# tensorboy/pytorch_Realtime_Multi-Person_Pose_Estimation

Hardware: AMD Instinct MI355X
Metric: end-to-end persons-posed FPS at 368x368 (net+pafprocess) (higher is better)
Workload: dtype fp32; 1 GPU; rtpose VGG19 368x368 batch=32 synthetic images, single MI355X, fp32 (BASELINE.json configs[1]); per-GPU batch 32, one process per GPU; global_batch=32, weights=seeded He init (no checkpoint offline), decoder_input=synthetic scene + 1e-3 * net output (blend kernel timed), humans_per_batch=163, parallelism=single GPU

## Files before the change

### pytorch_realtime_multi-person_pose_estimation_amd/csrc/conv_wino4.hip

```cpp
#include <hip/hip_runtime.h>

#include <cmath>
#include <cstdio>
#include <cstdlib>
#include <type_traits>

#include "conv_desc.h"
#include "launchers.h"
#include "wino_common.h"

namespace rtpose {

namespace wino4 {

using namespace winoc;

constexpr int W4_L0 = 6;

typedef float floatx4 __attribute__((ext_vector_type(4)));

struct Group {
  const float* in;
  const float* w;
  const float* bias;
  float* out;
  int in_cstride, in_choff, in_ws, in_hs, in_lead;
  int out_cstride, out_choff, out_ws, out_hs, out_lead;
  int cout, cout_pad;
  int in_pq, out_pq;
  size_t in_bytes, w_bytes, out_bytes;
};

__device__ __forceinline__ int px_floats(int cstride, int pq) { return pq ? 8 : cstride; }
__device__ __forceinline__ size_t ch0_floats(int choff, int pq) { return pq ? (size_t)(choff >> 3) * pq * 8 + (choff & 7) : choff; }
__device__ __forceinline__ unsigned col_floats(int col, int pq) { return pq ? (unsigned)(col >> 3) * pq * 8 + (col & 7) : col; }

struct Args {
  Group g[2];
  int N, H, W;
  int TY, TX, T;
  int cin;
  int relu, pool;
  int mtiles, ntiles, ncombo, xcd_remap;
  int persist;
  int mt0;
};

struct ArgsP : Args {
  const float* prelu[2];
};
template <bool PR>
using ArgsT = typename std::conditional<PR, ArgsP, Args>::type;
template <bool PR>
__device__ __forceinline__ float slope_of(const ArgsT<PR>& A, int grp, int ncol, int cout) {
  if constexpr (PR) return ncol < cout ? (grp ? A.prelu[1] : A.prelu[0])[ncol] : 0.f;
  return 0.f;
}

constexpr int NT = 32;
constexpr int NC = 64;
constexpr int CK = 8;
constexpr int NFP = 18;
constexpr int NPW = 9;
constexpr int NFW = 18;
constexpr int NB = 6;
constexpr int PF = 5;
constexpr int VBUF = NFP * 4 * NT;
constexpr int UBUF = 36 * 2 * NT;
static_assert((2 * NPW) % NB == 0, "the B ring rotates in step with two chunks");

template <class Out>
__device__ __forceinline__ void bt6(const F4 (&d)[6], Out out) {
  out(0, fma4(1.265625f, d[0], fma4(-2.8125f, d[2], d[4])));
  __builtin_amdgcn_sched_barrier(0);
  {
    const F4 e1 = fma4(-2.25f, d[2], d[4]), o1 = fma4(-2.25f, d[1], d[3]);
    out(1, fma4(0.75f, o1, e1));
    out(2, fma4(-0.75f, o1, e1));
  }
  __builtin_amdgcn_sched_barrier(0);
  {
    const F4 e2 = fma4(-0.5625f, d[2], d[4]), o2 = fma4(-0.5625f, d[1], d[3]);
    out(3, fma4(1.5f, o2, e2));
    out(4, fma4(-1.5f, o2, e2));
  }
  __builtin_amdgcn_sched_barrier(0);
  out(5, fma4(1.265625f, d[1], fma4(-2.8125f, d[3], d[5])));
}

__device__ __forceinline__ f2 splat(float s) { return f2{s, s}; }
__device__ __forceinline__ void at4_lo(const f2 (&m)[6], f2& y0, f2& y1) {
  const f2 s12 = m[1] + m[2], d12 = m[1] - m[2], s34 = m[3] + m[4], d34 = m[3] - m[4];
  y0 = (m[0] + s12) + s34;
  y1 = __builtin_elementwise_fma(splat(1.5f), d34, splat(0.75f) * d12);
}
__device__ __forceinline__ void at4_hi(const f2 (&m)[6], f2& y2, f2& y3) {
  const f2 s12 = m[1] + m[2], d12 = m[1] - m[2], s34 = m[3] + m[4], d34 = m[3] - m[4];
  y2 = __builtin_elementwise_fma(splat(2.25f), s34, splat(0.5625f) * s12);
  y3 = __builtin_elementwise_fma(splat(3.375f), d34, splat(0.421875f) * d12) + m[5];
}

template <int RT, bool PR = false>
__global__ __launch_bounds__(512, 1) void wino4_f32(const ArgsT<PR> A) {
  constexpr int NT = 16 * RT;
  constexpr int VBUF = NFP * 4 * NT;
  constexpr int UBUF = 36 * 2 * NT;
  extern __shared__ __attribute__((aligned(16))) float4 L4[];
  auto Vb = [&](int i) -> float4* { return L4 + i * (VBUF + UBUF); };
  auto Ub = [&](int i) -> float4* { return L4 + (1 - i) * (VBUF + UBUF) + VBUF; };
  const int tid = threadIdx.x;
  const int lane = tid & 63;
  const int wv = __builtin_amdgcn_readfirstlane(tid >> 6);
  const int wn = wv & 3, fh = wv >> 2;
  const int r16 = lane & 15, kq = lane >> 4;

  const int bi = blockIdx.x;
  int j0, jstep, c;
  if (A.persist) {
    const int xcd = bi & 7, idx = bi >> 3;
    c = idx % A.ncombo;
    j0 = (idx / A.ncombo) * 8 + xcd;
    jstep = gridDim.x / A.ncombo;
  } else {
    if (A.xcd_remap) {
      const int xcd = bi & 7, j = bi >> 3;
      c = j % A.ncombo;
      j0 = (j / A.ncombo) * 8 + xcd;
    } else {
      j0 = bi % A.mtiles;
      c = bi / A.mtiles;
    }
    jstep = A.mtiles;
  }
  if (j0 >= A.mtiles) return;
  const int nt = c % A.ntiles, grp = c / A.ntiles;
  const Group g = grp ? A.g[1] : A.g[0];
  const int TT = A.TY * A.TX;

  const bool s1 = RT == 2 ? wv < 6 : wv < 3, s2 = RT == 2 ? wv >= 2 : (wv >= 3 && wv < 6);
  const int turn = wv >> 2;
  const int wl1 = RT == 2 ? lane >> 1 : (lane >> 1) & 15, cg1 = lane & 1;
  const int wl = RT == 2 ? lane & 31 : lane & 15, cg = RT == 2 ? lane >> 5 : (lane >> 4) & 1;
  const int py = RT == 2 ? wv : 2 * (s1 ? wv : 0) + (lane >> 5);
  const int fx = RT == 2 ? max(wv - 2, 0) : 2 * (s2 ? wv - 3 : 0) + (lane >> 5);
  const i32x4 rw = make_rsrc(g.w, g.w_bytes);
  const i32x4 rnull = make_rsrc(g.in, 0);
  i32x4 rin;
  unsigned pv[4];
  int lt = j0, lc = 3;
  const int cs_ld = px_floats(g.in_cstride, g.in_pq);
  const unsigned pxb = (unsigned)cs_ld * 4;
  const unsigned ckb = g.in_pq ? (unsigned)g.in_pq * (CK * 4) : CK * 4;
  const size_t in_ch0 = ch0_floats(g.in_choff, g.in_pq);
  auto set_loader = [&](int mt, i32x4& r_, unsigned (&v_)[4]) {
    size_t q0;
    {
      const int t = min((A.mt0 + mt) * NT, A.T - 1);
      const int n = t / TT, r = t - n * TT;
      const int ty = r / A.TX, tx = r - ty * A.TX;
      q0 = (size_t)g.in_lead + (size_t)(n * g.in_hs + 4 * ty - 1) * g.in_ws + (4 * tx - 1);
    }
    const int t = min((A.mt0 + mt) * NT + wl1, A.T - 1);
    const int n = t / TT, r = t - n * TT;
    const int ty = r / A.TX, tx = r - ty * A.TX;
    const int yy = min(4 * ty - 1 + py, A.H);
    const size_t qq = (size_t)g.in_lead + (size_t)(n * g.in_hs + yy) * g.in_ws + (4 * tx - 1);
    const size_t o0 = q0 * cs_ld + in_ch0;
    r_ = make_rsrc(g.in + o0, g.in_bytes - o0 * 4);
    v_[0] = (unsigned)(((qq - q0) * cs_ld + cg1 * 4) * 4);
#pragma unroll
    for (int n5 = 3; n5 < 6; ++n5) v_[n5 - 2] = v_[0] + (unsigned)min(n5, A.W + 1 - 4 * tx) * pxb;
  };
  F4 p[6];
  auto load_piece = [&](const i32x4& r_, const unsigned (&v_)[4], int chunk, int n5) {
    const unsigned cb = (unsigned)chunk * ckb;
    p[n5] = n5 < 3 ? bload(r_, v_[0], cb + n5 * pxb) : bload(r_, v_[n5 - 2], cb);
  };
  const int ust = (py * 2 + cg1) * NT + (wl1 ^ (4 * cg1));
  const int uld = ((fx * 6) * 2 + cg) * NT + (wl ^ (4 * cg));
  const int vst = ((fx * 3) * 4 + 2 * cg) * NT + wl;
  auto stage1 = [&](int ubuf) {
    float4* dst = Ub(ubuf) + ust;
    bt6(p, [&](int f, F4 u) { dst[f * 6 * 2 * NT] = to_float4(u); });
  };
  F4 q[6];
  auto stage2_read = [&](int ubuf) {
    const float4* src = Ub(ubuf) + uld;
#pragma unroll
    for (int y = 0; y < 6; ++y) {
      const float4 t = src[y * 2 * NT];
      q[y] = F4{f2{t.x, t.y}, f2{t.z, t.w}};
    }
  };
  auto stage2 = [&](int vbuf) {
    float4* dst = Vb(vbuf) + vst;
    F4 ev;
    bt6(q, [&](int f, F4 v) {
      if (f & 1) {
        dst[(f >> 1) * 4 * NT] = make_float4(ev.lo.x, ev.lo.y, v.lo.x, v.lo.y);
        dst[(f >> 1) * 4 * NT + NT] = make_float4(ev.hi.x, ev.hi.y, v.hi.x, v.hi.y);
      } else {
        ev = v;
      }
    });
  };

  const int ncol = nt * NC + wn * 16 + r16;
  floatx4 acc[NFW][RT];
  const float bias0 = g.bias[ncol];
  const float slope0 = slope_of<PR>(A, grp, ncol, g.cout);
  const unsigned boff = (unsigned)((kq * g.cout_pad + ncol) * 16);
  const unsigned fstep = (unsigned)(4 * g.cout_pad * 16);
  const unsigned wbase = (unsigned)fh * (NPW * fstep);
  unsigned wso = wbase;
  float4 bs[NB];
  const int nchunks = A.cin / CK;
  const int aoff = fh * NPW * 4 * NT + kq * NT + r16;

  set_loader(j0, rin, pv);
#pragma unroll
  for (int i = 0; i < 6; ++i) load_piece(rin, pv, 0, i);
  if (s1) stage1(0);
#pragma unroll
  for (int i = 0; i < 6; ++i) load_piece(rin, pv, 1, i);
#pragma unroll
  for (int f = 0; f < PF; ++f) {
    bs[f] = bload_f4(rw, boff, wso);
    wso += fstep;
  }
  __syncthreads();
  stage2_read(0);
  if (s2) stage2(0);
  if (s1) stage1(1);
#pragma unroll
  for (int i = 0; i < 6; ++i) load_piece(rin, pv, 2, i);
  __syncthreads();

#define RTPOSE_PIN()             \
  asm volatile("" ::: "memory"); \
  __builtin_amdgcn_sched_barrier(0)
  for (int mt = j0; mt < A.mtiles; mt += jstep) {
#pragma unroll
    for (int f = 0; f < NFW; ++f)
#pragma unroll
      for (int rt = 0; rt < RT; ++rt)
#pragma unroll
        for (int v = 0; v < 4; ++v) acc[f][rt][v] = 0.f;

    float4 a0, a1;
#pragma unroll 1
    for (int c2 = 0; c2 < nchunks; c2 += 2) {
#pragma unroll
      for (int h = 0; h < 2; ++h) {
        const float4* va = Vb(h) + aoff;
        if (lc == nchunks) {
          lc = 0;
          lt += jstep;
          if (lt < A.mtiles) set_loader(lt, rin, pv);
        }
        const int c3 = lc++;
        const i32x4 rl = s1 ? rin : rnull;
        a0 = va[RT == 2 ? fh * 16 : 0];
        if (RT == 2) a1 = va[(fh ^ 1) * 16];
#pragma unroll
        for (int i = 0; i < NPW; ++i) {
          const float4 bv = bs[(h * NPW + i) % NB];
          acc[2 * i][0] = __builtin_amdgcn_mfma_f32_16x16x4f32(a0.x, bv.x, acc[2 * i][0], 0, 0, 0);
          acc[2 * i + 1][0] = __builtin_amdgcn_mfma_f32_16x16x4f32(a0.z, bv.z, acc[2 * i + 1][0], 0, 0, 0);
          acc[2 * i][0] = __builtin_amdgcn_mfma_f32_16x16x4f32(a0.y, bv.y, acc[2 * i][0], 0, 0, 0);
          acc[2 * i + 1][0] = __builtin_amdgcn_mfma_f32_16x16x4f32(a0.w, bv.w, acc[2 * i + 1][0], 0, 0, 0);
          RTPOSE_PIN();
          if (i < NPW - 1) a0 = va[(i + 1) * 4 * NT + (RT == 2 ? fh * 16 : 0)];
          {
            const int L = h * NPW + i + PF;
            bs[L % NB] = bload_f4(rw, boff, wso);
            if (L % NPW == NPW - 1) wso = (c2 + L / NPW == nchunks - 1) ? wbase : wso + (NPW + 1) * fstep;
            else wso += fstep;
          }
          RTPOSE_PIN();
          if (RT == 2) {
            acc[2 * i][RT - 1] = __builtin_amdgcn_mfma_f32_16x16x4f32(a1.x, bv.x, acc[2 * i][RT - 1], 0, 0, 0);
            acc[2 * i + 1][RT - 1] = __builtin_amdgcn_mfma_f32_16x16x4f32(a1.z, bv.z, acc[2 * i + 1][RT - 1], 0, 0, 0);
            acc[2 * i][RT - 1] = __builtin_amdgcn_mfma_f32_16x16x4f32(a1.y, bv.y, acc[2 * i][RT - 1], 0, 0, 0);
            acc[2 * i + 1][RT - 1] = __builtin_amdgcn_mfma_f32_16x16x4f32(a1.w, bv.w, acc[2 * i + 1][RT - 1], 0, 0, 0);
          }
          RTPOSE_PIN();
          if (RT == 2 && i < NPW - 1) a1 = va[(i + 1) * 4 * NT + (fh ^ 1) * 16];
          if (i < 2) {
            if (s1 && i == turn) stage1(h);
          } else if (i < 4) {
            if (i == 2 + turn) stage2_read(h ^ 1);
          } else if (i < 6) {
            if (s2 && i == 4 + turn) stage2(h ^ 1);
          }
          if (i >= W4_L0 && i < W4_L0 + 3) {
            load_piece(rl, pv, c3, 2 * (i - W4_L0));
            load_piece(rl, pv, c3, 2 * (i - W4_L0) + 1);
          }
          RTPOSE_PIN();
        }
        __syncthreads();
      }
    }

    f2 sk[3][RT][4], sr[3][RT][4];
    if (RT == 2) {
      float4* const E = L4 + VBUF + UBUF;
#pragma unroll
      for (int vp = 0; vp < RT; ++vp) {
        f2 sg[3][4];
#pragma unroll
        for (int xl = 0; xl < 3; ++xl) {
          f2 m[6];
#pragma unroll
          for (int y = 0; y < 6; ++y) m[y] = f2{acc[xl * 6 + y][RT - 1][2 * vp], acc[xl * 6 + y][RT - 1][2 * vp + 1]};
          at4_lo(m, sg[xl][0], sg[xl][1]);
          at4_hi(m, sg[xl][2], sg[xl][3]);
        }
#pragma unroll
        for (int xl = 0; xl < 3; ++xl)
#pragma unroll
          for (int hh = 0; hh < 2; ++hh)
            E[(wv * 6 + xl * 2 + hh) * 64 + lane] =
                make_float4(sg[xl][2 * hh].x, sg[xl][2 * hh].y, sg[xl][2 * hh + 1].x, sg[xl][2 * hh + 1].y);
#pragma unroll
        for (int xl = 0; xl < 3; ++xl) {
          f2 m[6];
#pragma unroll
          for (int y = 0; y < 6; ++y) m[y] = f2{acc[xl * 6 + y][0][2 * vp], acc[xl * 6 + y][0][2 * vp + 1]};
          at4_lo(m, sk[xl][vp][0], sk[xl][vp][1]);
          at4_hi(m, sk[xl][vp][2], sk[xl][vp][3]);
        }
        __syncthreads();
#pragma unroll
        for (int xl = 0; xl < 3; ++xl)
#pragma unroll
          for (int hh = 0; hh < 2; ++hh) {
            const float4 t = E[((wv ^ 4) * 6 + xl * 2 + hh) * 64 + lane];
            sr[xl][vp][2 * hh] = f2{t.x, t.y};
            sr[xl][vp][2 * hh + 1] = f2{t.z, t.w};
          }
        __syncthreads();
      }
    } else {
      float4* const E = L4;
      auto rowsums = [&](int pair, f2 (&dst)[3][RT][4]) {
#pragma unroll
        for (int xl = 0; xl < 3; ++xl) {
          f2 m[6];
#pragma unroll
          for (int y = 0; y < 6; ++y)
            m[y] = pair ? f2{acc[xl * 6 + y][0][2], acc[xl * 6 + y][0][3]} : f2{acc[xl * 6 + y][0][0], acc[xl * 6 + y][0][1]};
          at4_lo(m, dst[xl][0][0], dst[xl][0][1]);
          at4_hi(m, dst[xl][0][2], dst[xl][0][3]);
        }
      };
      rowsums(fh ^ 1, sr);
#pragma unroll
      for (int xl = 0; xl < 3; ++xl)
#pragma unroll
        for (int hh = 0; hh < 2; ++hh)
          E[(wv * 6 + xl * 2 + hh) * 64 + lane] =
              make_float4(sr[xl][0][2 * hh].x, sr[xl][0][2 * hh].y, sr[xl][0][2 * hh + 1].x, sr[xl][0][2 * hh + 1].y);
      rowsums(fh, sk);
      __syncthreads();
#pragma unroll
      for (int xl = 0; xl < 3; ++xl)
#pragma unroll
        for (int hh = 0; hh < 2; ++hh) {
          const float4 t = E[((wv ^ 4) * 6 + xl * 2 + hh) * 64 + lane];
          sr[xl][0][2 * hh] = f2{t.x, t.y};
          sr[xl][0][2 * hh + 1] = f2{t.z, t.w};
        }
    }
    auto finish = [&](auto fhc) {
      constexpr int FH = decltype(fhc)::value;
      auto S = [&](int x, int vp, int i) -> f2 { return (x / 3 == FH) ? sk[x % 3][vp][i] : sr[x % 3][vp][i]; };
      const bool col_ok = ncol < g.cout;
      const int sc = A.pool ? 2 : 4;
      auto wt_q = [&](int n, int ty, int tx) -> int { return (n * g.out_hs + sc * ty) * g.out_ws + sc * tx; };
      int q0;
      {
        const int t = min((A.mt0 + mt) * NT, A.T - 1);
        const int n = t / TT, r = t - n * TT;
        const int ty = r / A.TX;
        q0 = wt_q(n, ty, r - ty * A.TX);
      }
      const int cs_st = px_floats(g.out_cstride, g.out_pq);
      const size_t oo0 = ((size_t)g.out_lead + (size_t)q0) * cs_st + ch0_floats(g.out_choff, g.out_pq);
      const i32x4 rout = make_rsrc(g.out + oo0, g.out_bytes - oo0 * 4);
      const unsigned cs4 = (unsigned)cs_st * 4, row4 = (unsigned)g.out_ws * cs4;
      const unsigned col4 = col_floats(ncol, g.out_pq) * 4;
      int tcur = (A.mt0 + mt) * NT + (RT == 2 ? FH * 16 + 4 * kq : 4 * kq + 2 * FH);
      int sn = tcur / TT, sy, sx;
      {
        const int r = tcur - sn * TT;
        sy = r / A.TX;
        sx = r - sy * A.TX;
      }
#pragma unroll
      for (int vp = 0; vp < RT; ++vp) {
        unsigned off[2];
        bool okv[2];
        int ylim[2], xlim[2];
#pragma unroll
        for (int e = 0; e < 2; ++e) {
          okv[e] = col_ok && tcur < A.T;
          off[e] = (unsigned)(wt_q(sn, sy, sx) - q0) * cs4 + col4;
          ylim[e] = A.H - 4 * sy;
          xlim[e] = A.W - 4 * sx;
          ++tcur;
          const bool wx = sx + 1 >= A.TX, wy = wx && sy + 1 >= A.TY;
          sx = wx ? 0 : sx + 1;
          sy = wy ? 0 : (wx ? sy + 1 : sy);
          sn += wy ? 1 : 0;
        }
#pragma unroll
        for (int ih = 0; ih < 2; ++ih) {
          f2 yy[2][4];
#pragma unroll
          for (int il = 0; il < 2; ++il) {
            f2 m[6];
#pragma unroll
            for (int x = 0; x < 6; ++x) m[x] = S(x, vp, 2 * ih + il);
            at4_lo(m, yy[il][0], yy[il][1]);
            at4_hi(m, yy[il][2], yy[il][3]);
          }
          if (A.pool) {
#pragma unroll
            for (int jh = 0; jh < 2; ++jh) {
              f2 mx = __builtin_elementwise_max(__builtin_elementwise_max(yy[0][2 * jh], yy[0][2 * jh + 1]),
                                                __builtin_elementwise_max(yy[1][2 * jh], yy[1][2 * jh + 1]));
              mx = mx + splat(bias0);
              if (A.relu) mx = __builtin_elementwise_max(mx, splat(0.f));
#pragma unroll
              for (int e = 0; e < 2; ++e) {
                const bool ok = okv[e] && 2 * ih < ylim[e] && 2 * jh < xlim[e];
                bstore(mx[e], rout, ok ? off[e] : kNoStore, ih * row4 + jh * cs4);
              }
            }
          } else {
#pragma unroll
            for (int il = 0; il < 2; ++il)
#pragma unroll
              for (int j = 0; j < 4; ++j) {
                const int i = 2 * ih + il;
                f2 o = yy[il][j] + splat(bias0);
                if (A.relu) o = __builtin_elementwise_max(o, splat(0.f));
                if constexpr (PR) {
                  o[0] = prelu1(o[0], slope0);
                  o[1] = prelu1(o[1], slope0);
                }
#pragma unroll
                for (int e = 0; e < 2; ++e) {
                  const bool ok = okv[e] && i < ylim[e] && j < xlim[e];
                  bstore(o[e], rout, ok ? off[e] : kNoStore, i * row4 + j * cs4);
                }
              }
          }
        }
      }
    };
    if (fh == 0) finish(std::integral_constant<int, 0>{});
    else finish(std::integral_constant<int, 1>{});
  }
#undef RTPOSE_PIN
}

constexpr int NTS = 16;
constexpr int VBUFS = NFP * 4 * NTS;
constexpr int UBUFS = 36 * 2 * NTS;

template <bool PR = false>
__global__ __launch_bounds__(384, 2) void wino4s_f32(const ArgsT<PR> A) {
  extern __shared__ __attribute__((aligned(16))) float4 L4[];
  auto Vb = [&](int i) -> float4* { return L4 + i * VBUFS; };
  auto Ub = [&](int i) -> float4* { return L4 + 2 * VBUFS + i * UBUFS; };
  const int tid = threadIdx.x;
  const int lane = tid & 63;
  const int wv = __builtin_amdgcn_readfirstlane(tid >> 6);
  const int r16 = lane & 15, kq = lane >> 4;

  const int bi = blockIdx.x;
  const int mt = A.mt0 + bi % A.mtiles, c = bi / A.mtiles;
  const int nt = c % A.ntiles, grp = c / A.ntiles;
  const Group g = grp ? A.g[1] : A.g[0];
  const int TT = A.TY * A.TX;
  const int nchunks = A.cin / CK;

  const bool s1 = wv < 3;
  const int hi5 = lane >> 5;
  const int wl1 = (lane >> 1) & 15, cg1 = lane & 1, py = 2 * (s1 ? wv : 0) + hi5;
  const int wl = lane & 15, cg = (lane >> 4) & 1, fx = 2 * (s1 ? 0 : wv - 3) + hi5;
  const i32x4 rw = make_rsrc(g.w, g.w_bytes);
  i32x4 rin;
  unsigned pv0, pvx;
  const int cs_ld = px_floats(g.in_cstride, g.in_pq);
  const unsigned pxb = (unsigned)cs_ld * 4;
  const unsigned ckb = g.in_pq ? (unsigned)g.in_pq * (CK * 4) : CK * 4;
  {
    size_t q0;
    {
      const int t = min(mt * NTS, A.T - 1);
      const int n = t / TT, r = t - n * TT;
      const int ty = r / A.TX, tx = r - ty * A.TX;
      q0 = (size_t)g.in_lead + (size_t)(n * g.in_hs + 4 * ty - 1) * g.in_ws + (4 * tx - 1);
    }
    const int t = min(mt * NTS + wl1, A.T - 1);
    const int n = t / TT, r = t - n * TT;
    const int ty = r / A.TX, tx = r - ty * A.TX;
    const int yy = min(4 * ty - 1 + py, A.H);
    const size_t qq = (size_t)g.in_lead + (size_t)(n * g.in_hs + yy) * g.in_ws + (4 * tx - 1);
    const size_t o0 = q0 * cs_ld + ch0_floats(g.in_choff, g.in_pq);
    rin = make_rsrc(g.in + o0, s1 ? g.in_bytes - o0 * 4 : 0);
    pv0 = (unsigned)(((qq - q0) * cs_ld + cg1 * 4) * 4);
    pvx = (unsigned)(A.W + 1 - 4 * tx);
  }
  F4 p[6];
  auto load_piece = [&](int chunk, int n5) {
    const unsigned cb = (unsigned)min(chunk, nchunks - 1) * ckb;
    p[n5] = n5 < 3 ? bload(rin, pv0, cb + n5 * pxb) : bload(rin, pv0 + min((unsigned)n5, pvx) * pxb, cb);
  };
  const int ust = (py * 2 + cg1) * NTS + (wl1 ^ (4 * cg1));
  const int uld = ((fx * 6) * 2 + cg) * NTS + (wl ^ (4 * cg));
  const int vst = ((fx * 3) * 4 + 2 * cg) * NTS + wl;
  auto stage1 = [&](int ubuf) {
    float4* dst = Ub(ubuf) + ust;
    bt6(p, [&](int f, F4 u) { dst[f * 6 * 2 * NTS] = to_float4(u); });
  };
  F4 q[6];
  auto stage2_read = [&](int ubuf) {
    const float4* src = Ub(ubuf) + uld;
#pragma unroll
    for (int y = 0; y < 6; ++y) {
      const float4 t = src[y * 2 * NTS];
      q[y] = F4{f2{t.x, t.y}, f2{t.z, t.w}};
    }
  };
  auto stage2 = [&](int vbuf) {
    float4* dst = Vb(vbuf) + vst;
    F4 ev;
    bt6(q, [&](int f, F4 v) {
      if (f & 1) {
        dst[(f >> 1) * 4 * NTS] = make_float4(ev.lo.x, ev.lo.y, v.lo.x, v.lo.y);
        dst[(f >> 1) * 4 * NTS + NTS] = make_float4(ev.hi.x, ev.hi.y, v.hi.x, v.hi.y);
      } else {
        ev = v;
      }
    });
  };

  const int ncol = nt * 16 + r16;
  floatx4 acc[6];
#pragma unroll
  for (int f = 0; f < 6; ++f)
#pragma unroll
    for (int v = 0; v < 4; ++v) acc[f][v] = 0.f;
  const unsigned boff = (unsigned)((kq * g.cout_pad + ncol) * 16);
  const unsigned fstep = (unsigned)(4 * g.cout_pad * 16);
  unsigned wso = (unsigned)wv * 3 * fstep;
  float4 bs[6];
  const int aoff = wv * 3 * 4 * NTS + kq * NTS + r16;

#pragma unroll
  for (int i = 0; i < 6; ++i) load_piece(0, i);
  if (s1) stage1(0);
#pragma unroll
  for (int i = 0; i < 6; ++i) load_piece(1, i);
#pragma unroll
  for (int i = 0; i < 3; ++i) {
    bs[i] = bload_f4(rw, boff, wso);
    wso += fstep;
  }
  wso += (NFP - 3) * fstep;
  __syncthreads();
  if (!s1) {
    stage2_read(0);
    stage2(0);
  }
  if (s1) stage1(1);
#pragma unroll
  for (int i = 0; i < 6; ++i) load_piece(2, i);
  __syncthreads();

#pragma unroll 1
  for (int c2 = 0; c2 < nchunks; c2 += 2) {
#pragma unroll
    for (int h = 0; h < 2; ++h) {
      const float4* va = Vb(h) + aoff;
#pragma unroll
      for (int i = 0; i < 3; ++i) {
        bs[((h ^ 1) * 3) + i] = bload_f4(rw, boff, wso);
        wso += fstep;
      }
      wso += (NFP - 3) * fstep;
      if (s1) stage1(h);
      else stage2_read(h ^ 1);
#pragma unroll
      for (int i = 0; i < 6; ++i) load_piece(c2 + h + 3, i);
#pragma unroll
      for (int i = 0; i < 3; ++i) {
        const float4 av = va[i * 4 * NTS], bv = bs[h * 3 + i];
        acc[2 * i] = __builtin_amdgcn_mfma_f32_16x16x4f32(av.x, bv.x, acc[2 * i], 0, 0, 0);
        acc[2 * i + 1] = __builtin_amdgcn_mfma_f32_16x16x4f32(av.z, bv.z, acc[2 * i + 1], 0, 0, 0);
        acc[2 * i] = __builtin_amdgcn_mfma_f32_16x16x4f32(av.y, bv.y, acc[2 * i], 0, 0, 0);
        acc[2 * i + 1] = __builtin_amdgcn_mfma_f32_16x16x4f32(av.w, bv.w, acc[2 * i + 1], 0, 0, 0);
      }
      if (!s1) stage2(h ^ 1);
      __syncthreads();
    }
  }

  {
    float4* const E = L4;
#pragma unroll
    for (int vp = 0; vp < 2; ++vp) {
      f2 m[6], sg[4];
#pragma unroll
      for (int y = 0; y < 6; ++y) m[y] = f2{acc[y][2 * vp], acc[y][2 * vp + 1]};
      at4_lo(m, sg[0], sg[1]);
      at4_hi(m, sg[2], sg[3]);
#pragma unroll
      for (int hh = 0; hh < 2; ++hh)
        E[((wv * 2 + vp) * 2 + hh) * 64 + lane] = make_float4(sg[2 * hh].x, sg[2 * hh].y, sg[2 * hh + 1].x, sg[2 * hh + 1].y);
    }
    __syncthreads();
    if (wv < 4) {
      const int vp = wv >> 1, ih = wv & 1;
      f2 sl[6][2];
#pragma unroll
      for (int x = 0; x < 6; ++x) {
        const float4 t = E[((x * 2 + vp) * 2 + ih) * 64 + lane];
        sl[x][0] = f2{t.x, t.y};
        sl[x][1] = f2{t.z, t.w};
      }
      const bool col_ok = ncol < g.cout;
      const float bias0 = g.bias[ncol];
      float slope0 = 0.f;
      if constexpr (PR) slope0 = slope_of<PR>(A, grp, ncol, g.cout);
      const int sc = A.pool ? 2 : 4;
      auto wt_q = [&](int n, int ty, int tx) -> int { return (n * g.out_hs + sc * ty) * g.out_ws + sc * tx; };
      int q0;
      {
        const int t = min(mt * NTS, A.T - 1);
        const int n = t / TT, r = t - n * TT;
        const int ty = r / A.TX;
        q0 = wt_q(n, ty, r - ty * A.TX);
      }
      const int cs_st = px_floats(g.out_cstride, g.out_pq);
      const size_t oo0 = ((size_t)g.out_lead + (size_t)q0) * cs_st + ch0_floats(g.out_choff, g.out_pq);
      const i32x4 rout = make_rsrc(g.out + oo0, g.out_bytes - oo0 * 4);
      const unsigned cs4 = (unsigned)cs_st * 4, row4 = (unsigned)g.out_ws * cs4;
      const unsigned col4 = col_floats(ncol, g.out_pq) * 4;
      unsigned off[2];
      bool okv[2];
      int ylim[2], xlim[2];
#pragma unroll
      for (int e = 0; e < 2; ++e) {
        const int tcur = mt * NTS + 4 * kq + 2 * vp + e;
        const int sn = tcur / TT, r = tcur - sn * TT;
        const int sy = r / A.TX, sx = r - sy * A.TX;
        okv[e] = col_ok && tcur < A.T;
        off[e] = (unsigned)(wt_q(sn, sy, sx) - q0) * cs4 + col4;
        ylim[e] = A.H - 4 * sy;
        xlim[e] = A.W - 4 * sx;
      }
      f2 yy[2][4];
#pragma unroll
      for (int il = 0; il < 2; ++il) {
        f2 m[6];
#pragma unroll
        for (int x = 0; x < 6; ++x) m[x] = sl[x][il];
        at4_lo(m, yy[il][0], yy[il][1]);
        at4_hi(m, yy[il][2], yy[il][3]);
      }
      if (A.pool) {
#pragma unroll
        for (int jh = 0; jh < 2; ++jh) {
          f2 mx = __builtin_elementwise_max(__builtin_elementwise_max(yy[0][2 * jh], yy[0][2 * jh + 1]),
                                            __builtin_elementwise_max(yy[1][2 * jh], yy[1][2 * jh + 1]));
          mx = mx + splat(bias0);
          if (A.relu) mx = __builtin_elementwise_max(mx, splat(0.f));
#pragma unroll
          for (int e = 0; e < 2; ++e) {
            const bool ok = okv[e] && 2 * ih < ylim[e] && 2 * jh < xlim[e];
            bstore(mx[e], rout, ok ? off[e] : kNoStore, ih * row4 + jh * cs4);
          }
        }
      } else {
#pragma unroll
        for (int il = 0; il < 2; ++il)
#pragma unroll
          for (int j = 0; j < 4; ++j) {
            const int i = 2 * ih + il;
            f2 o = yy[il][j] + splat(bias0);
            if (A.relu) o = __builtin_elementwise_max(o, splat(0.f));
            if constexpr (PR) {
              o[0] = prelu1(o[0], slope0);
              o[1] = prelu1(o[1], slope0);
            }
#pragma unroll
            for (int e = 0; e < 2; ++e) {
              const bool ok = okv[e] && i < ylim[e] && j < xlim[e];
              bstore(o[e], rout, ok ? off[e] : kNoStore, i * row4 + j * cs4);
            }
          }
      }
    }
  }
}

__device__ __forceinline__ double g43(int f, int k) {
  const double G[6][3] = {{64.0 / 81.0, 0.0, 0.0},
                          {-128.0 / 243.0, -32.0 / 81.0, -8.0 / 27.0},
                          {-128.0 / 243.0, 32.0 / 81.0, -8.0 / 27.0},
                          {32.0 / 243.0, 16.0 / 81.0, 8.0 / 27.0},
                          {32.0 / 243.0, -16.0 / 81.0, 8.0 / 27.0},
                          {0.0, 0.0, 1.0}};
  return G[f][k];
}
__device__ __forceinline__ double u43(const float* gw, int fxi, int fyi) {
  double v = 0.0;
#pragma unroll
  for (int ky = 0; ky < 3; ++ky)
#pragma unroll
    for (int kx = 0; kx < 3; ++kx) v += g43(fyi, ky) * g43(fxi, kx) * (double)gw[ky * 3 + kx];
  return v;
}

__global__ void pack_wino4_kernel(const float* __restrict__ w, const float* __restrict__ bias, int cout, int cin_src,
                                  const int32_t* __restrict__ cin_map, int cin_packed, int coutp,
                                  float* __restrict__ wp, float* __restrict__ bp) {
  const size_t total = (size_t)36 * cin_packed * coutp;
  const size_t i = (size_t)blockIdx.x * blockDim.x + threadIdx.x;
  if (i < (size_t)coutp) bp[i] = (i < (size_t)cout && bias) ? bias[i] : 0.f;
  if (i >= total) return;
  const int e = i & 1, fh = (i >> 1) & 1;
  size_t r = i >> 2;
  const int n = r % coutp;
  r /= coutp;
  const int kq = r & 3;
  r >>= 2;
  const int fp = r % NFP;
  const int chunk = r / NFP;
  const int cc = chunk * CK + 2 * kq + e;
  const int src = cin_map ? cin_map[cc] : (cc < cin_src ? cc : -1);
  float v = 0.f;
  if (n < cout && src >= 0 && src < cin_src) {
    const int f = 2 * fp + fh;
    v = (float)u43(w + ((size_t)n * cin_src + src) * 9, f / 6, f % 6);
  }
  wp[i] = v;
}

__global__ void wino4_amp_kernel(const float* __restrict__ w, int cout, int cin, float* __restrict__ amp) {
  __shared__ float red[37][256];
  const int o = blockIdx.x, tid = threadIdx.x;
  float sf[36], den = 0.f;
#pragma unroll
  for (int f = 0; f < 36; ++f) sf[f] = 0.f;
  for (int cidx = tid; cidx < cin; cidx += 256) {
    const float* gw = w + ((size_t)o * cin + cidx) * 9;
    for (int k = 0; k < 9; ++k) den += fabsf(gw[k]);
#pragma unroll
    for (int f = 0; f < 36; ++f) sf[f] += fabsf((float)u43(gw, f / 6, f % 6));
  }
#pragma unroll
  for (int f = 0; f < 36; ++f) red[f][tid] = sf[f];
  red[36][tid] = den;
  __syncthreads();
  for (int st = 128; st > 0; st >>= 1) {
    if (tid < st)
      for (int f = 0; f < 37; ++f) red[f][tid] += red[f][tid + st];
    __syncthreads();
  }
  if (tid == 0) {
    const float at[4][6] = {{1.f, 1.f, 1.f, 1.f, 1.f, 0.f},
                            {0.f, 0.75f, 0.75f, 1.5f, 1.5f, 0.f},
                            {0.f, 0.5625f, 0.5625f, 2.25f, 2.25f, 0.f},
                            {0.f, 0.421875f, 0.421875f, 3.375f, 3.375f, 1.f}};
    const float bsum[6] = {5.078125f, 5.6875f, 5.6875f, 3.90625f, 3.90625f, 5.078125f};
    float num = 0.f;
    for (int i = 0; i < 4; ++i)
      for (int j = 0; j < 4; ++j) {
        float v = 0.f;
        for (int fxi = 0; fxi < 6; ++fxi)
          for (int fyi = 0; fyi < 6; ++fyi) v += at[i][fyi] * at[j][fxi] * bsum[fyi] * bsum[fxi] * red[fxi * 6 + fyi][0];
        num = fmaxf(num, v);
      }
    const float r = red[36][0] > 0.f ? num / red[36][0] : 0.f;
    atomicMax(reinterpret_cast<int*>(amp), __float_as_int(r));
  }
}

}

int conv2d_wino4_ok(int cin, int cout) { return cout > 0 && cin % 16 == 0 && cin >= 32; }

size_t packed_weight_floats_wino4(int cout, int cin) { return (size_t)36 * cin * cout_pad(cout); }

namespace {
template <bool PR>
int wino4_run(wino4::ArgsT<PR> a, long ids, int ngroups, int cout0, hipStream_t s) {
  using namespace wino4;
  const int n_cu = device_cu_count();
  auto launch_small = [&](const ArgsT<PR>& a0, int mt0_32, long wtiles) -> int {
    ArgsT<PR> b = a0;
    b.persist = 0;
    b.mt0 = 2 * mt0_32;
    b.mtiles = (int)((wtiles + NTS - 1) / NTS);
    b.ntiles = cout_pad(cout0) / 16;
    b.ncombo = b.ntiles * ngroups;
    return launch_kernel<wino4s_f32<PR>>(dim3((unsigned)((long)b.mtiles * b.ncombo)), dim3(384),
                                         (size_t)(2 * VBUFS + 2 * UBUFS) * sizeof(float4), 80 * 1024, s, b);
  };
  auto launch_half = [&](const ArgsT<PR>& a0, int mt0_32, long wtiles) -> int {
    ArgsT<PR> b = a0;
    b.persist = 0;
    b.mt0 = 2 * mt0_32;
    b.mtiles = (int)((wtiles + 15) / 16);
    long idh;
    if (int rc = grid_ids(b.mtiles, b.ncombo, b.xcd_remap, idh, "conv2d_winograd (4x4)")) return rc;
    return launch_kernel<wino4_f32<1, PR>>(dim3((unsigned)idh), dim3(512), (size_t)(VBUF + UBUF) * sizeof(float4), 150 * 1024,
                                           s, b);
  };
  if ((long)a.mtiles * a.ncombo * 2 <= n_cu) return launch_small(a, 0, a.T);
  int rest = 0;
  bool rest_half = false;
  if ((long)a.mtiles * a.ncombo > n_cu && n_cu % (8 * a.ncombo) == 0) {
    const int Pc = n_cu / a.ncombo;
    const int r = a.mtiles % Pc;
    if (r && (long)r * a.ncombo * 4 <= n_cu) {
      rest = r;
      a.mtiles -= r;
    } else if (r && 2L * r * a.ncombo <= n_cu) {
      rest = r;
      rest_half = true;
      a.mtiles -= r;
    }
    a.persist = 1;
    ids = n_cu;
  }
  if (int rc = launch_kernel<wino4_f32<2, PR>>(dim3((unsigned)ids), dim3(512), (size_t)(2 * VBUF + 2 * UBUF) * sizeof(float4),
                                               150 * 1024, s, a))
    return rc;
  if (rest && rest_half) return launch_half(a, a.mtiles, (long)a.T - (long)a.mtiles * NT);
  if (rest) return launch_small(a, a.mtiles, (long)a.T - (long)a.mtiles * NT);
  return 0;
}
}

int conv2d_wino4_launch(const rtpose_conv_desc* d, int ngroups, int N, int H, int W, hipStream_t s) {
  using namespace wino4;
  const ConvSpec spec = {"conv2d_winograd (4x4)", 4, 1, false, true, true, true};
  if (int rc = check_conv_features(d, ngroups, spec)) return rc;
  const rtpose_conv_desc& d0 = d[0];
  if (d0.k != 3 || !conv2d_wino4_ok(d0.cin, d0.cout))
    return fail(RTPOSE_E_INVAL, "%s: k must be 3 and cin a multiple of 16, >= 32", spec.who);
  if (int rc = check_conv_layouts(d, ngroups, N, H, W, spec)) return rc;
  Args a;
  memset(&a, 0, sizeof(a));
  for (int i = 0; i < ngroups; ++i) {
    const rtpose_conv_desc& di = d[i];
    if (di.in_plane_pixels < 0 || di.out_plane_pixels < 0 ||
        (di.in_plane_pixels && ((di.lin.choff % 8) || (size_t)di.in_plane_pixels < rtpose_layout_pixels(&di.lin, N, H, W))) ||
        (di.out_plane_pixels &&
         ((di.lout.choff % 8) || (di.cout % 8) ||
          (size_t)di.out_plane_pixels < rtpose_layout_pixels(&di.lout, N, di.pool ? H / 2 : H, di.pool ? W / 2 : W))))
      return fail(RTPOSE_E_INVAL, "%s: channel-plane slices start at a multiple of 8 channels (the output "
                                  "has a multiple of 8 of them) and a plane holds at least the layout's pixels", spec.who);
    if ((di.in_plane_pixels && (size_t)(di.lin.choff + di.cin) / 8 * di.in_plane_pixels * 32 > (size_t)winoc::kMaxRange) ||
        (di.out_plane_pixels && (size_t)(di.lout.choff + cout_pad(di.cout)) / 8 * di.out_plane_pixels * 32 > (size_t)winoc::kMaxRange))
      return fail(RTPOSE_E_INVAL, "%s: channel-plane slice beyond 2 GiB", spec.who);
    Group& g = a.g[i];
    fill_group(g, di);
    g.in_pq = di.in_plane_pixels;
    g.out_pq = di.out_plane_pixels;
    g.in_bytes = g.in_pq ? (size_t)(di.lin.choff + di.cin) / 8 * g.in_pq * 32
                         : rtpose_layout_pixels(&di.lin, N, H, W) * (size_t)di.lin.cstride * sizeof(float);
    g.w_bytes = packed_weight_floats_wino4(di.cout, di.cin) * sizeof(float);
    g.out_bytes = g.out_pq ? (size_t)(di.lout.choff + di.cout) / 8 * g.out_pq * 32
                           : rtpose_layout_pixels(&di.lout, N, di.pool ? H / 2 : H, di.pool ? W / 2 : W) *
                                 (size_t)di.lout.cstride * sizeof(float);
  }
  a.N = N;
  a.H = H;
  a.W = W;
  a.TY = ceil_div(H, 4);
  a.TX = ceil_div(W, 4);
  const long T = (long)N * a.TY * a.TX;
  if (T > 0x7fffffffL) return fail(RTPOSE_E_INVAL, "%s: tensor too large", spec.who);
  a.T = (int)T;
  a.cin = d0.cin;
  a.relu = d0.relu;
  a.pool = d0.pool;
  a.mtiles = ceil_div(a.T, NT);
  a.ntiles = cout_pad(d0.cout) / NC;
  a.ncombo = a.ntiles * ngroups;
  long ids;
  if (int rc = grid_ids(a.mtiles, a.ncombo, a.xcd_remap, ids, spec.who)) return rc;
  if (!d0.prelu) return wino4_run<false>(a, ids, ngroups, d0.cout, s);
  ArgsP ap;
  static_cast<Args&>(ap) = a;
  set_prelu(ap, d, ngroups);
  return wino4_run<true>(ap, ids, ngroups, d0.cout, s);
}

int pack_weights_wino4_launch(const float* w, const float* bias, int cout, int cin_src, const int32_t* cin_map,
                              int cin_packed, float* wp, float* bp, hipStream_t s) {
  if (!conv2d_wino4_ok(cin_packed, cout) || (cin_packed < cin_src && !cin_map))
    return fail(RTPOSE_E_INVAL, "pack_winograd (4x4): cin_packed must be a multiple of 16, >= 32 and >= cin_src");
  const int coutp = cout_pad(cout);
  const size_t total = (size_t)36 * cin_packed * coutp;
  const int threads = 256;
  const unsigned blocks = (unsigned)((total + threads - 1) / threads);
  hipLaunchKernelGGL(wino4::pack_wino4_kernel, dim3(blocks), dim3(threads), 0, s, w, bias, cout, cin_src, cin_map,
                     cin_packed, coutp, wp, bp);
  RTPOSE_HIP_CHECK(hipGetLastError());
  return 0;
}

int wino4_amplification_launch(const float* w, int cout, int cin, float* amp, hipStream_t s) {
  hipLaunchKernelGGL(wino4::wino4_amp_kernel, dim3(cout), dim3(256), 0, s, w, cout, cin, amp);
  RTPOSE_HIP_CHECK(hipGetLastError());
  return 0;
}

double conv2d_wino4_issued_flops(int cin, int cout, int N, int H, int W) {
  const double T = (double)N * ceil_div(H, 4) * ceil_div(W, 4);
  const double tiles = std::ceil(T / 32.0);
  return 2.0 * tiles * 32.0 * 36.0 * (double)cin * cout_pad(cout);
}

}
```

Measured before the change: 1449 images/s.

## Add wide 16-byte output stores via quad DPP transpose in wino4 epilogue

Adds a WD template variant of the 4x4 Winograd kernel. Each lane quad transposes its outputs with DPP quad permutes, so one 16-byte buffer store writes four consecutive channels in place of four scalar stores per element; the pooled path packs its 2x2 max outputs the same way. The variant is selected at launch when cout, output alignment and channel strides are multiples of four and PReLU is off. The change also recomputes lane indices and bias via mbcnt to shorten register live ranges, and uses a scalar-register buffer descriptor with 32-bit offset math in the RT=2 loader. The risks are extra DPP/select instructions, an added s_nop after each store, and a second kernel instantiation.

After: 1453 images/s (median of 6 runs). Within noise of the previous version (+0.3%).

```diff
diff --git a/pytorch_realtime_multi-person_pose_estimation_amd/csrc/conv_wino4.hip b/pytorch_realtime_multi-person_pose_estimation_amd/csrc/conv_wino4.hip
--- a/pytorch_realtime_multi-person_pose_estimation_amd/csrc/conv_wino4.hip
+++ b/pytorch_realtime_multi-person_pose_estimation_amd/csrc/conv_wino4.hip
@@ -100,7 +100,44 @@
   y3 = __builtin_elementwise_fma(splat(3.375f), d34, splat(0.421875f) * d12) + m[5];
 }
 
-template <int RT, bool PR = false>
+__device__ __forceinline__ int lane_now() {
+  int l;
+  asm volatile("v_mbcnt_lo_u32_b32 %0, -1, 0\n\tv_mbcnt_hi_u32_b32 %0, -1, %0" : "=v"(l));
+  return l;
+}
+__device__ __forceinline__ i32x4 make_rsrc_s(const void* p, size_t bytes) {
+  i32x4 r = make_rsrc(p, 0);
+  unsigned hi = (unsigned)(bytes >> 32);
+  asm("" : "+s"(hi));
+  r[2] = (int)(hi ? kMaxRange : min((unsigned)bytes, kMaxRange));
+  return r;
+}
+
+__device__ void llvm_raw_buffer_store_v4f32(f32x4 v, i32x4 rsrc, int voffset, int soffset, int aux) __asm(
+    "llvm.amdgcn.raw.buffer.store.v4f32");
+template <int CTRL>
+__device__ __forceinline__ float quad_perm(float v) {
+  return __builtin_bit_cast(float, __builtin_amdgcn_update_dpp(0, __builtin_bit_cast(int, v), CTRL, 0xf, 0xf, true));
+}
+__device__ __forceinline__ void quad_transpose(float (&r)[4], int q) {
+  constexpr int X1 = 0xb1, X2 = 0x4e;
+  const bool odd = q & 1, hi = q & 2;
+  const float a0 = quad_perm<X1>(r[0]), a1 = quad_perm<X1>(r[1]), a2 = quad_perm<X1>(r[2]), a3 = quad_perm<X1>(r[3]);
+  const float x0 = odd ? a1 : r[0], x1 = odd ? r[1] : a0, x2 = odd ? a3 : r[2], x3 = odd ? r[3] : a2;
+  const float b0 = quad_perm<X2>(x0), b1 = quad_perm<X2>(x1), b2 = quad_perm<X2>(x2), b3 = quad_perm<X2>(x3);
+  r[0] = hi ? b2 : x0;
+  r[2] = hi ? x2 : b0;
+  r[1] = hi ? b3 : x1;
+  r[3] = hi ? x3 : b1;
+}
+__device__ __forceinline__ void bstore4(const float (&r)[4], i32x4 rs, unsigned voff, unsigned soff) {
+  llvm_raw_buffer_store_v4f32(f32x4{r[0], r[1], r[2], r[3]}, rs, (int)voff, (int)soff, 0);
+  __builtin_amdgcn_sched_barrier(0);
+  asm volatile("s_nop 1");
+  __builtin_amdgcn_sched_barrier(0);
+}
+
+template <int RT, bool PR = false, bool WD = false>
 __global__ __launch_bounds__(512, 1) void wino4_f32(const ArgsT<PR> A) {
   constexpr int NT = 16 * RT;
   constexpr int VBUF = NFP * 4 * NT;
@@ -160,14 +197,25 @@
       const int ty = r / A.TX, tx = r - ty * A.TX;
       q0 = (size_t)g.in_lead + (size_t)(n * g.in_hs + 4 * ty - 1) * g.in_ws + (4 * tx - 1);
     }
-    const int t = min((A.mt0 + mt) * NT + wl1, A.T - 1);
+    int wl1_ = wl1, cg1_ = cg1;
+    if constexpr (RT == 2) {
+      const int l = lane_now();
+      wl1_ = l >> 1;
+      cg1_ = l & 1;
+    }
+    const int t = min((A.mt0 + mt) * NT + wl1_, A.T - 1);
     const int n = t / TT, r = t - n * TT;
     const int ty = r / A.TX, tx = r - ty * A.TX;
     const int yy = min(4 * ty - 1 + py, A.H);
     const size_t qq = (size_t)g.in_lead + (size_t)(n * g.in_hs + yy) * g.in_ws + (4 * tx - 1);
     const size_t o0 = q0 * cs_ld + in_ch0;
-    r_ = make_rsrc(g.in + o0, g.in_bytes - o0 * 4);
-    v_[0] = (unsigned)(((qq - q0) * cs_ld + cg1 * 4) * 4);
+    if constexpr (RT == 2) {
+      r_ = make_rsrc_s(g.in + o0, g.in_bytes - o0 * 4);
+      v_[0] = ((unsigned)(qq - q0) * (unsigned)cs_ld + (unsigned)cg1_ * 4) * 4;
+    } else {
+      r_ = make_rsrc(g.in + o0, g.in_bytes - o0 * 4);
+      v_[0] = (unsigned)(((qq - q0) * cs_ld + cg1 * 4) * 4);
+    }
 #pragma unroll
     for (int n5 = 3; n5 < 6; ++n5) v_[n5 - 2] = v_[0] + (unsigned)min(n5, A.W + 1 - 4 * tx) * pxb;
   };
@@ -304,8 +352,12 @@
     }
 
     f2 sk[3][RT][4], sr[3][RT][4];
+    float bias_t = bias0, slope_t = slope0;
     if (RT == 2) {
       float4* const E = L4 + VBUF + UBUF;
+      const int le = lane_now();
+      bias_t = g.bias[nt * NC + wn * 16 + (le & 15)];
+      if constexpr (PR) slope_t = slope_of<PR>(A, grp, nt * NC + wn * 16 + (le & 15), g.cout);
 #pragma unroll
       for (int vp = 0; vp < RT; ++vp) {
         f2 sg[3][4];
@@ -321,7 +373,7 @@
         for (int xl = 0; xl < 3; ++xl)
 #pragma unroll
           for (int hh = 0; hh < 2; ++hh)
-            E[(wv * 6 + xl * 2 + hh) * 64 + lane] =
+            E[(wv * 6 + xl * 2 + hh) * 64 + le] =
                 make_float4(sg[xl][2 * hh].x, sg[xl][2 * hh].y, sg[xl][2 * hh + 1].x, sg[xl][2 * hh + 1].y);
 #pragma unroll
         for (int xl = 0; xl < 3; ++xl) {
@@ -336,7 +388,7 @@
         for (int xl = 0; xl < 3; ++xl)
 #pragma unroll
           for (int hh = 0; hh < 2; ++hh) {
-            const float4 t = E[((wv ^ 4) * 6 + xl * 2 + hh) * 64 + lane];
+            const float4 t = E[((wv ^ 4) * 6 + xl * 2 + hh) * 64 + le];
             sr[xl][vp][2 * hh] = f2{t.x, t.y};
             sr[xl][vp][2 * hh + 1] = f2{t.z, t.w};
           }
@@ -376,6 +428,8 @@
     auto finish = [&](auto fhc) {
       constexpr int FH = decltype(fhc)::value;
       auto S = [&](int x, int vp, int i) -> f2 { return (x / 3 == FH) ? sk[x % 3][vp][i] : sr[x % 3][vp][i]; };
+      const int lf = lane_now();
+      const int kq = lf >> 4, ncol = nt * NC + wn * 16 + (lf & 15);
       const bool col_ok = ncol < g.cout;
       const int sc = A.pool ? 2 : 4;
       auto wt_q = [&](int n, int ty, int tx) -> int { return (n * g.out_hs + sc * ty) * g.out_ws + sc * tx; };
@@ -391,6 +445,9 @@
       const i32x4 rout = make_rsrc(g.out + oo0, g.out_bytes - oo0 * 4);
       const unsigned cs4 = (unsigned)cs_st * 4, row4 = (unsigned)g.out_ws * cs4;
       const unsigned col4 = col_floats(ncol, g.out_pq) * 4;
+      constexpr bool wide = WD;
+      const int q4 = lf & 3;
+      const unsigned colq4 = col_floats(ncol & ~3, g.out_pq) * 4 + (A.pool ? (q4 >> 1) * row4 + (q4 & 1) * cs4 : q4 * cs4);
       int tcur = (A.mt0 + mt) * NT + (RT == 2 ? FH * 16 + 4 * kq : 4 * kq + 2 * FH);
       int sn = tcur / TT, sy, sx;
       {
@@ -400,13 +457,14 @@
       }
 #pragma unroll
       for (int vp = 0; vp < RT; ++vp) {
-        unsigned off[2];
+        unsigned off[2], offq[2];
         bool okv[2];
         int ylim[2], xlim[2];
 #pragma unroll
         for (int e = 0; e < 2; ++e) {
           okv[e] = col_ok && tcur < A.T;
           off[e] = (unsigned)(wt_q(sn, sy, sx) - q0) * cs4 + col4;
+          offq[e] = (unsigned)(wt_q(sn, sy, sx) - q0) * cs4 + colq4;
           ylim[e] = A.H - 4 * sy;
           xlim[e] = A.W - 4 * sx;
           ++tcur;
@@ -415,6 +473,7 @@
           sy = wy ? 0 : (wx ? sy + 1 : sy);
           sn += wy ? 1 : 0;
         }
+        f2 pm[2][2];
 #pragma unroll
         for (int ih = 0; ih < 2; ++ih) {
           f2 yy[2][4];
@@ -431,8 +490,10 @@
             for (int jh = 0; jh < 2; ++jh) {
               f2 mx = __builtin_elementwise_max(__builtin_elementwise_max(yy[0][2 * jh], yy[0][2 * jh + 1]),
                                                 __builtin_elementwise_max(yy[1][2 * jh], yy[1][2 * jh + 1]));
-              mx = mx + splat(bias0);
+              mx = mx + splat(bias_t);
               if (A.relu) mx = __builtin_elementwise_max(mx, splat(0.f));
+              pm[ih][jh] = mx;
+              if constexpr (wide) continue;
 #pragma unroll
               for (int e = 0; e < 2; ++e) {
                 const bool ok = okv[e] && 2 * ih < ylim[e] && 2 * jh < xlim[e];
@@ -441,22 +502,45 @@
             }
           } else {
 #pragma unroll
-            for (int il = 0; il < 2; ++il)
+            for (int il = 0; il < 2; ++il) {
+              const int i = 2 * ih + il;
+              f2 o[4];
 #pragma unroll
               for (int j = 0; j < 4; ++j) {
-                const int i = 2 * ih + il;
-                f2 o = yy[il][j] + splat(bias0);
-                if (A.relu) o = __builtin_elementwise_max(o, splat(0.f));
+                o[j] = yy[il][j] + splat(bias_t);
+                if (A.relu) o[j] = __builtin_elementwise_max(o[j], splat(0.f));
                 if constexpr (PR) {
-                  o[0] = prelu1(o[0], slope0);
-                  o[1] = prelu1(o[1], slope0);
-                }
-#pragma unroll
-                for (int e = 0; e < 2; ++e) {
-                  const bool ok = okv[e] && i < ylim[e] && j < xlim[e];
-                  bstore(o[e], rout, ok ? off[e] : kNoStore, i * row4 + j * cs4);
+                  o[j][0] = prelu1(o[j][0], slope_t);
+                  o[j][1] = prelu1(o[j][1], slope_t);
                 }
               }
+              if constexpr (wide) {
+#pragma unroll
+                for (int e = 0; e < 2; ++e) {
+                  float r[4] = {o[0][e], o[1][e], o[2][e], o[3][e]};
+                  quad_transpose(r, q4);
+                  const bool ok = okv[e] && i < ylim[e] && q4 < xlim[e];
+                  bstore4(r, rout, ok ? offq[e] : kNoStore, i * row4);
+                }
+              } else {
+#pragma unroll
+                for (int j = 0; j < 4; ++j)
+#pragma unroll
+                  for (int e = 0; e < 2; ++e) {
+                    const bool ok = okv[e] && i < ylim[e] && j < xlim[e];
+                    bstore(o[j][e], rout, ok ? off[e] : kNoStore, i * row4 + j * cs4);
+                  }
+              }
+            }
+          }
+        }
+        if (wide && A.pool) {
+#pragma unroll
+          for (int e = 0; e < 2; ++e) {
+            float r[4] = {pm[0][0][e], pm[0][1][e], pm[1][0][e], pm[1][1][e]};
+            quad_transpose(r, q4);
+            const bool ok = okv[e] && (q4 & 2) < ylim[e] && 2 * (q4 & 1) < xlim[e];
+            bstore4(r, rout, ok ? offq[e] : kNoStore, 0);
           }
         }
       }
@@ -804,6 +888,11 @@
 int wino4_run(wino4::ArgsT<PR> a, long ids, int ngroups, int cout0, hipStream_t s) {
   using namespace wino4;
   const int n_cu = device_cu_count();
+  bool wd = !PR;
+  for (int i = 0; i < ngroups; ++i) {
+    const Group& g = a.g[i];
+    wd = wd && g.cout % 4 == 0 && ((size_t)g.out & 15) == 0 && (g.out_pq || ((g.out_choff | g.out_cstride) & 3) == 0);
+  }
   auto launch_small = [&](const ArgsT<PR>& a0, int mt0_32, long wtiles) -> int {
     ArgsT<PR> b = a0;
     b.persist = 0;
@@ -821,8 +910,10 @@
     b.mtiles = (int)((wtiles + 15) / 16);
     long idh;
     if (int rc = grid_ids(b.mtiles, b.ncombo, b.xcd_remap, idh, "conv2d_winograd (4x4)")) return rc;
-    return launch_kernel<wino4_f32<1, PR>>(dim3((unsigned)idh), dim3(512), (size_t)(VBUF + UBUF) * sizeof(float4), 150 * 1024,
-                                           s, b);
+    const size_t lds = (size_t)(VBUF + UBUF) * sizeof(float4);
+    if constexpr (!PR)
+      if (wd) return launch_kernel<wino4_f32<1, false, true>>(dim3((unsigned)idh), dim3(512), lds, 150 * 1024, s, b);
+    return launch_kernel<wino4_f32<1, PR>>(dim3((unsigned)idh), dim3(512), lds, 150 * 1024, s, b);
   };
   if ((long)a.mtiles * a.ncombo * 2 <= n_cu) return launch_small(a, 0, a.T);
   int rest = 0;
@@ -841,9 +932,13 @@
     a.persist = 1;
     ids = n_cu;
   }
-  if (int rc = launch_kernel<wino4_f32<2, PR>>(dim3((unsigned)ids), dim3(512), (size_t)(2 * VBUF + 2 * UBUF) * sizeof(float4),
-                                               150 * 1024, s, a))
-    return rc;
+  const size_t lds = (size_t)(2 * VBUF + 2 * UBUF) * sizeof(float4);
+  auto launch_big = [&]() -> int {
+    if constexpr (!PR)
+      if (wd) return launch_kernel<wino4_f32<2, false, true>>(dim3((unsigned)ids), dim3(512), lds, 150 * 1024, s, a);
+    return launch_kernel<wino4_f32<2, PR>>(dim3((unsigned)ids), dim3(512), lds, 150 * 1024, s, a);
+  };
+  if (int rc = launch_big()) return rc;
   if (rest && rest_half) return launch_half(a, a.mtiles, (long)a.T - (long)a.mtiles * NT);
   if (rest) return launch_small(a, a.mtiles, (long)a.T - (long)a.mtiles * NT);
   return 0;
```
